# dkouzoup/ms-eetc

Hardware: NVIDIA B200
Metric: OCP solves/sec (batched, 1/2/4/8 B200) vs CasADi+IPOPT on host cores (higher is better)
Workload: dtype f64

## Files before the change

ms-eetc_b200/csrc/mseetc_b200.cu:

```cuda
#include <cuda_runtime.h>
#include <cooperative_groups.h>

#include <algorithm>
#include <cstdio>
#include <limits>
#include <cstdlib>
#include <cstring>
#include <new>
#include <string>
#include <vector>

#include "../../include/mseetc_b200.h"
#include "variants.h"
#include "compact.cuh"
#include "table.cuh"

using namespace mseetc;

static_assert((int)MSEETC_PARAM_COUNT == (int)PAR_N, "parameter plane enum out of sync");
static_assert((int)MSEETC_P_MASS == (int)P_MASS, "parameter plane enum out of sync");

namespace {

thread_local std::string g_err;


#ifndef MS_MINB_TRIAL
#define MS_MINB_TRIAL 2
#endif
#ifndef MS_MINB_EVAL
#define MS_MINB_EVAL 2
#endif
#ifndef MS_MINB_STEP
#define MS_MINB_STEP 3
#endif
MS_CELL_KERNEL(k_cell_setup, 4, cell_setup(c, io, k, s))
MS_CELL_KERNEL(k_cell_init, 4, cell_init<false>(c, k, s))
MS_CELL_KERNEL(k_cell_trial_eval, MS_MINB_TRIAL, (cell_eval<false, true>(c, k, s)))
MS_CELL_KERNEL(k_cell_eval, MS_MINB_EVAL, (cell_eval<false, false>(c, k, s)))
MS_CELL_KERNEL(k_cell_step, MS_MINB_STEP, cell_step<false>(c, k, s))
MS_CELL_KERNEL(k_cell_extract, 4, cell_extract(c, io, k, s))

__global__ void __launch_bounds__(64) k_inst_setup(Ctx c, BatchIO io) {
    const int s = blockIdx.x * blockDim.x + threadIdx.x;
    if (s < c.cfg.S) inst_setup(c, io, s);
}
__global__ void __launch_bounds__(128) k_inst_profile(Ctx c, int useSmem) {
    extern __shared__ double prof_sm[];
    const int half = blockDim.x >> 1;
    const bool profileRole = (int)threadIdx.x >= half;
    const int col = profileRole ? (int)threadIdx.x - half : (int)threadIdx.x;
    const int s = blockIdx.x * half + col;
    if (s >= c.cfg.S) return;
    if (!profileRole) { inst_screen(c, s); return; }
    if (useSmem) inst_profile(c, s, prof_sm + col, prof_sm + (size_t)c.cfg.NK * half + col, half);
    else inst_profile(c, s);
}

#ifndef MS_RED_CL
#define MS_RED_CL 4
#endif
enum { RED_CL = MS_RED_CL, RED_WB = RED_W / RED_CL };
static_assert(RED_W % RED_CL == 0, "cluster size must divide the interleave factor");
__device__ __forceinline__ const double* cluster_peer(const double* p, unsigned rank) {
    return cooperative_groups::this_cluster().map_shared_rank(p, rank);
}
__device__ __forceinline__ void prefetch_instance_state(const Ctx& c, int s) {
    for (int f = 0; f < SD_N; ++f) asm volatile("prefetch.global.L1 [%0];" ::"l"(&c.D(f, s)));
    for (int f = 0; f < SI_N; ++f) asm volatile("prefetch.global.L1 [%0];" ::"l"(&c.I(f, s)));
}

__global__ void __cluster_dims__(RED_CL, 1, 1) __launch_bounds__(32 * RED_WB) k_inst_alpha(Ctx c, int* mirror) {
    namespace cg = cooperative_groups;
    cg::cluster_group cl = cg::this_cluster();
    if (mirror && blockIdx.x == 0 && threadIdx.x == 0) *mirror = *(volatile int*)c.done;
    __shared__ double sm[RED_WB][3][32];
    const unsigned rank = cl.block_rank();
    const int lane = threadIdx.x & 31, wl = threadIdx.x >> 5, w = (int)rank * RED_WB + wl;
    const int s = (blockIdx.x / RED_CL) * 32 + lane;
    const bool on = s < c.cfg.nInst && c.I(SI_PHASE, s) == PH_STEPPED;
    double acc[3] = {1.0, 1.0, 0.0};
    if (on) alpha_partials(c, s, c.I(SI_N_INT, s), w, RED_W, acc);
    if (on && rank == 0 && wl == 0) prefetch_instance_state(c, s);
    for (int f = 0; f < 3; ++f) sm[wl][f][lane] = acc[f];
    cl.sync();
    double tot[3] = {1.0, 1.0, 0.0};
    if (rank == 0 && wl == 0 && on) {
        for (int ww = 0; ww < RED_W; ++ww) {
            const double* q = cluster_peer(&sm[ww % RED_WB][0][lane], ww / RED_WB);
            tot[0] = fmin(tot[0], q[0]); tot[1] = fmin(tot[1], q[32]); tot[2] += q[64];
        }
    }
    cl.sync();
    if (rank == 0 && wl == 0 && on) inst_alpha(c, s, tot);
}

template <bool TRIAL>
__global__ void __cluster_dims__(RED_CL, 1, 1) __launch_bounds__(32 * RED_WB) k_inst_kkt(Ctx c) {
    namespace cg = cooperative_groups;
    cg::cluster_group cl = cg::this_cluster();
    __shared__ double sm[RED_WB][10][32];
    const unsigned rank = cl.block_rank();
    const int lane = threadIdx.x & 31, wl = threadIdx.x >> 5, w = (int)rank * RED_WB + wl;
    const int s = (blockIdx.x / RED_CL) * 32 + lane;
    const bool on = s < c.cfg.nInst && c.I(SI_PHASE, s) == (TRIAL ? PH_TRIAL : PH_EVAL);
    KktAcc acc;
    kkt_init(acc);
    if (on) kkt_partials(c, s, c.I(SI_N_INT, s), ((c.I(SI_PARITY, s) != 0) != TRIAL) ? WS_IT1 : WS_IT0, w, RED_W, acc);
    if (on && rank == 0 && wl == 0) prefetch_instance_state(c, s);
    sm[wl][0][lane] = acc.th; sm[wl][1][lane] = acc.fo; sm[wl][2][lane] = acc.slog; sm[wl][3][lane] = acc.sdamp;
    sm[wl][4][lane] = acc.zsum; sm[wl][5][lane] = acc.ysum; sm[wl][6][lane] = acc.dinf; sm[wl][7][lane] = acc.pinf;
    sm[wl][8][lane] = acc.cmin; sm[wl][9][lane] = acc.cmax;
    cl.sync();
    KktAcc tot;
    kkt_init(tot);
    const bool lead = rank == 0 && wl == 0 && on;
    if (lead) {
        for (int ww = 0; ww < RED_W; ++ww) {
            const double* q = cluster_peer(&sm[ww % RED_WB][0][lane], ww / RED_WB);
            KktAcc o;
            o.th = q[0]; o.fo = q[32]; o.slog = q[64]; o.sdamp = q[96];
            o.zsum = q[128]; o.ysum = q[160]; o.dinf = q[192]; o.pinf = q[224];
            o.cmin = q[256]; o.cmax = q[288];
            kkt_combine(tot, o);
        }
    }
    cl.sync();
    if (lead) {
        if (TRIAL) {
            const double sums[4] = {tot.th, tot.fo, tot.slog, tot.sdamp};
            inst_decide(c, s, sums);
        } else count_cells(c, 4, c.I(SI_N_INT, s) + 1);
        inst_kkt(c, s, tot);
    }
}

template <int BS, int DEPTH, bool BULK>
__global__ void __launch_bounds__(BS) k_step(Ctx c) {
    extern __shared__ __align__(128) double ring[];
    const int s = blockIdx.x * BS + threadIdx.x;
    if (s >= c.cfg.S) return;
    const int lane = threadIdx.x & 31, warp = threadIdx.x >> 5;
    const bool active = s < c.cfg.nInst && c.I(SI_PHASE, s) == PH_FACTOR;
    double* wring = ring + (size_t)warp * ((DEPTH + 1) * RING_NF_MAX * 32);
    if (BULK) {
        const unsigned mask = __ballot_sync(0xffffffffu, active);
        if (!active) return;
        const int N = c.I(SI_N_INT, s);
        if (__all_sync(mask, N == __shfl_sync(mask, N, __ffs((int)mask) - 1))) {
            unsigned long long* bars = reinterpret_cast<unsigned long long*>(ring + (size_t)(BS / 32) * ((DEPTH + 1) * RING_NF_MAX * 32))
                                       + (size_t)warp * 2 * (DEPTH + 1);
            BulkRing<BwdFields, DEPTH> fb;
            BulkRing<FwdFields, DEPTH> ff;
            fb.setup(wring, bars, mask, lane);
            ff.setup(wring, bars + (DEPTH + 1), mask, lane);
            inst_step_warp(c, s, mask, fb, ff);
            return;
        }
    }
    if (!active) return;
    RingFetch<BwdFields, 32, DEPTH> fb;
    fb.sm = wring + lane;
    RingFetch<FwdFields, 32, DEPTH> ff;
    ff.sm = wring + lane;
    inst_step(c, s, fb, ff);
}

#ifndef MS_PIT_PF
#define MS_PIT_PF 3
#endif
template <int SL, int G, int DEPTH>
__global__ void __launch_bounds__(SL * G) k_step_pit(Ctx c, int* fallbackCount) {
    extern __shared__ __align__(128) double pit_sm[];
    constexpr int BS = SL * G;
    double* ring = pit_sm;
    double* shbase = pit_sm + (size_t)(DEPTH + 1) * RING_NF_MAX * BS;
    int* flags = reinterpret_cast<int*>(shbase + (size_t)G * SH_N * SL);
    const int col = threadIdx.x % SL, l = threadIdx.x / SL;
    const int s = blockIdx.x * SL + col;
    const bool active = s < c.cfg.nInst && c.I(SI_PHASE, s) == PH_FACTOR;
    if (!__syncthreads_or(active)) return;
    PitShare sh{shbase, flags, SL};
    PitLane t;
    t.s = s; t.col = col; t.l = l; t.G = G;
    t.N = active ? c.I(SI_N_INT, s) : 2;
    t.mu = active ? c.D(SD_MU, s) : 0.1;
    t.delta = 0.0;
    const double dlast = active ? c.D(SD_DELTA_LAST, s) : 0.0;
    pit_chunk(t.N, G, l, t.kLo, t.kHi);
    if (active) pit_read_reference(c, t);
    if (l == 0) flags[col] = 0;
    RingFetch<BwdFields, BS, DEPTH, MS_PIT_PF> fb;
    fb.sm = ring + threadIdx.x;
    constexpr int FDEPTH = ((DEPTH + 1) * BwdFields::NF) / FwdFields::NF - 1;
    RingFetch<FwdFields, BS, FDEPTH, 2 * MS_PIT_PF> ff;
    ff.sm = ring + threadIdx.x;
    double delta = 0.0;
    bool pending = active, failed = false, fallback = false;
    int why = 0;
    for (int tries = 0; tries < 40; ++tries) {
        if (!__syncthreads_or(pending)) break;
        t.delta = delta;
        if (pending) {
            if (l == 0) count_cells(c, 2, t.N);
            pit_phase_a(c, t, sh, fb);
        }
        __syncthreads();
        if (pending && l == 0) pit_value_chain(sh, col, G);
        __syncthreads();
        if (pending) pit_phase_c(c, t, sh, fb);
        __syncthreads();
        const int f = flags[col];
        __syncthreads();
        if (l == 0) flags[col] = 0;
        if (pending) {
            if (f & PIT_SCAN_FAILED) { fallback = true; pending = false; why = f; }
            else if (f & PIT_BAD_INERTIA) {
                if (l == 0) c.I(SI_NREG, s) += 1;
                delta = pit_next_delta(delta, dlast);
                if (delta > 1e40) { failed = true; pending = false; }
            } else pending = false;
        }
    }
    if (pending) failed = true;
    if (__syncthreads_or(fallback)) {
        if (fallback && l == 0) {
            atomicAdd(fallbackCount, 1);
            if (why & PIT_ELEM_FAILED) atomicAdd(fallbackCount + 1, 1);
            if (why & PIT_APPLY_FAILED) atomicAdd(fallbackCount + 2, 1);
            if (why & PIT_INCONSISTENT) atomicAdd(fallbackCount + 3, 1);
            inst_step(c, s, fb, ff);
        }
        __syncthreads();
    }
    const bool go = active && !fallback && !failed;
    if (failed && l == 0) finish(c, s, ST_STEP_FAILED);
    if (go && l == 0) {
        pit_state_chain(sh, col, G);
        count_cells(c, 3, t.N);
        if (delta > 0.0) c.D(SD_DELTA_LAST, s) = delta;
        c.D(SD_DELTA, s) = delta;
    }
    __syncthreads();
    if (go) pit_phase_f(c, t, sh, ff);
    if (go && l == 0) { c.I(SI_FACT, s) = 1; c.I(SI_PHASE, s) = PH_STEPPED; }
}

__global__ void k_loop_cond(cudaGraphConditionalHandle handle, int* counters, int n, int maxTicks) {
    const int tick = ++counters[53];
    cudaGraphSetConditional(handle, (*(volatile int*)counters < n && tick <= maxTicks) ? 1u : 0u);
}

__global__ void __launch_bounds__(128) k_cell_table(TableIO io, LossMapDev lm) {
    const size_t total = (size_t)(io.Nmax + 1) * io.n;
    for (size_t idx = (size_t)blockIdx.x * 128 + threadIdx.x; idx < total; idx += (size_t)gridDim.x * 128)
        cell_table(io, lm, (int)(idx % (io.Nmax + 1)), (int)(idx / (io.Nmax + 1)));
// ... 315 lines not shown
        static const int stepDepth = []() { const char* e = getenv("MSEETC_STEP_DEPTH"); return e ? atoi(e) : 16; }();
        if (depth >= 16 && stepDepth >= 16 && !stepBulk) { depth = 16; stepKernel = k_step<32, 16, false>; }
        else if (depth >= 8) { depth = 8; stepKernel = stepBulk ? k_step<32, 8, true> : k_step<32, 8, false>; }
        else { depth = 4; stepKernel = k_step<32, 4, false>; }
    } else {
        if (depth >= 4) { depth = 4; stepKernel = k_step<64, 4, false>; }
        else if (depth >= 2) { depth = 2; stepKernel = k_step<64, 2, false>; }
        else { depth = 1; stepKernel = k_step<64, 1, false>; }
    }
    size_t ringBytes = (size_t)(depth + 1) * slotBytes + (size_t)(ib / 32) * 2 * (depth + 1) * sizeof(unsigned long long);
    static const int stepSmemKb = []() { const char* e = getenv("MSEETC_STEP_SMEM_KB"); return e ? atoi(e) : -1; }();
    {
        const int bps = blocksPerSm < 1 ? 1 : blocksPerSm;
        const size_t pad = stepSmemKb >= 0 ? (size_t)stepSmemKb * 1024 : (size_t)228 * 1024 / (bps + 1) + 1024;
        if (pad > ringBytes && pad <= (size_t)227 * 1024) ringBytes = pad;
    }
    cudaFuncSetAttribute(stepKernel, cudaFuncAttributeMaxDynamicSharedMemorySize, 227 * 1024);
    void (*pitKernel)(Ctx, int*) = nullptr;
    int pitThreads = 0, pitSL = 8;
    size_t pitBytes = 0;
    int lanesNow = h->sweep_lanes;
    if (lanesNow == 0) {
        const int Nmax = p.n_intervals_max;
        lanesNow = Nmax >= 1024 ? 32 : Nmax >= 96 ? 16 : Nmax >= 48 ? 8 : 1;
        if (lanesNow > 1 && lanesNow < 32 && g.S > 4096) lanesNow = 1;
    }
    h->last_lanes = lanesNow;
    if (lanesNow > 1) {
        const int G = lanesNow;
        pitSL = (G == 32) ? 8 : 16;
        if (G == 8) pitKernel = k_step_pit<16, 8, 1>;
        else if (G == 16) pitKernel = k_step_pit<16, 16, 1>;
        else pitKernel = k_step_pit<8, 32, 1>;
        pitThreads = pitSL * G;
        pitBytes = sizeof(double) * ((size_t)2 * RING_NF_MAX * pitThreads + (size_t)G * SH_N * pitSL) + sizeof(int) * pitSL;
        cudaFuncSetAttribute(pitKernel, cudaFuncAttributeMaxDynamicSharedMemorySize, 227 * 1024);
    }
    int launches = 0;
    cudaError_t e;
    for (int i = 0; i < NCLS; ++i) { h->ms[i] = 0.0; h->launches[i] = 0; h->cells[i] = 0; }
    std::vector<int> evClass;
    auto begin = [&](int cls) {
        h->launches[cls] += 1;
        ++launches;
        if (!h->profiling) return;
        const size_t need = 2 * (evClass.size() + 1);
        while (h->ev.size() < need) { cudaEvent_t x; cudaEventCreate(&x); h->ev.push_back(x); }
        cudaEventRecord(h->ev[2 * evClass.size()], st);
    };
    auto end = [&](int cls) {
        if (!h->profiling) return;
        cudaEventRecord(h->ev[2 * evClass.size() + 1], st);
        evClass.push_back(cls);
    };
    e = cudaMemsetAsync(c.done, 0, 256, st);
    if (e != cudaSuccess) return cuda_fail(e, "cudaMemsetAsync");
    e = cudaMemsetAsync(c.si, 0, sizeof(int) * (size_t)SI_N * g.S, st);
    if (e != cudaSuccess) return cuda_fail(e, "cudaMemsetAsync");
    const unsigned rgrid = (unsigned)(g.S / 32);
    begin(CLS_MISC); k_inst_setup<<<igrid, ib, 0, st>>>(c, io); end(CLS_MISC);
    begin(CLS_MISC); k_cell_setup<<<cgrid, 128, 0, st>>>(c, io); end(CLS_MISC);
    if (g.initMode || (tmin && g.energy)) {
        size_t profBytes = (size_t)2 * g.NK * ib * sizeof(double);
        if (profBytes > (size_t)200 * 1024 / (blocksPerSm < 1 ? 1 : blocksPerSm)) profBytes = 0;
        if (profBytes) cudaFuncSetAttribute(k_inst_profile, cudaFuncAttributeMaxDynamicSharedMemorySize, 227 * 1024);
        begin(CLS_MISC); k_inst_profile<<<igrid, 2 * ib, profBytes, st>>>(c, profBytes ? 1 : 0); end(CLS_MISC);
    }
    begin(CLS_MISC);
    if (intl) launch_variant(c.irk ? VK_INIT_INTL_IRK : VK_INIT_INTL, cgrid, st, c, io);
    else if (dyn) launch_variant(VK_INIT_DYN, cgrid, st, c, io); else k_cell_init<<<cgrid, 128, 0, st>>>(c, io);
    end(CLS_MISC);
    const int maxTicks = 3 * p.max_iterations + 100;
    int tick = 0;
    begin(CLS_EVAL);
    if (intl) launch_variant(c.irk ? VK_EVAL_INTL_IRK : VK_EVAL_INTL, gridIrk, st, c, io);
    else if (c.irk) launch_variant(dyn ? VK_EVAL_DYN_IRK : VK_EVAL_IRK, gridIrk, st, c, io);
    else if (dyn) launch_variant(VK_EVAL_DYN, gridEval, st, c, io); else k_cell_eval<<<gridEval, 128, 0, st>>>(c, io);
    end(CLS_EVAL);
    begin(CLS_KKT); k_inst_kkt<false><<<rgrid * RED_CL, 32 * RED_WB, 0, st>>>(c); end(CLS_KKT);
    static const bool compactOn = []() { const char* e = getenv("MSEETC_COMPACT"); return !e || atoi(e) != 0; }();
    h->last_compactions = 0;
    static const int graphEnv = []() { const char* e = getenv("MSEETC_GRAPH"); return e ? atoi(e) : -1; }();
    const bool useGraph = !h->profiling && (graphEnv == 1 || (graphEnv != 0 && g.S <= 256 && !tmin));
    auto tick_kernels = [&](cudaStream_t s0, int* mirror, bool prof) {
        if (prof) begin(CLS_STEP);
        if (pitKernel) pitKernel<<<(unsigned)(g.S / pitSL), pitThreads, pitBytes, s0>>>(c, c.done + 48);
        else stepKernel<<<igrid, ib, ringBytes, s0>>>(c);
        if (prof) end(CLS_STEP);
        if (prof) begin(CLS_CSTEP);
        if (intl) launch_variant(VK_STEP_INTL, pgrid(2), s0, c, io);
        else if (dyn) launch_variant(VK_STEP_DYN, gridStep, s0, c, io); else k_cell_step<<<gridStep, 128, 0, s0>>>(c, io);
        if (prof) end(CLS_CSTEP);
        if (prof) begin(CLS_ALPHA);
        k_inst_alpha<<<rgrid * RED_CL, 32 * RED_WB, 0, s0>>>(c, mirror);
        if (prof) end(CLS_ALPHA);
        if (prof) begin(CLS_TRIAL);
        if (intl) launch_variant(c.irk ? VK_TRIAL_INTL_IRK : VK_TRIAL_INTL, gridIrk, s0, c, io);
        else if (c.irk) launch_variant(dyn ? VK_TRIAL_DYN_IRK : VK_TRIAL_IRK, gridIrk, s0, c, io);
        else if (dyn) launch_variant(VK_TRIAL_DYN, gridTrial, s0, c, io); else k_cell_trial_eval<<<gridTrial, 128, 0, s0>>>(c, io);
        if (prof) end(CLS_TRIAL);
        if (prof) begin(CLS_DECIDE);
        k_inst_kkt<true><<<rgrid * RED_CL, 32 * RED_WB, 0, s0>>>(c);
        if (prof) end(CLS_DECIDE);
    };
    if (useGraph) {
        unsigned char key[sizeof h->loop_key];
        memset(key, 0, sizeof key);
        memcpy(key, &c, sizeof(Ctx));
        memcpy(key + sizeof(Ctx), &io, sizeof(BatchIO));
        int stPrio = 0;
        cudaStreamGetPriority(st, &stPrio);
        const int extra[4] = {lanesNow * 4 + (dyn ? 1 : 0), stPrio, maxTicks, n};
        memcpy(key + sizeof(Ctx) + sizeof(BatchIO), extra, sizeof extra);
        if (!h->loop_exec || memcmp(key, h->loop_key, sizeof key) != 0) {
            if (h->loop_exec) { cudaGraphExecDestroy(h->loop_exec); h->loop_exec = nullptr; }
            if (h->loop_graph) { cudaGraphDestroy(h->loop_graph); h->loop_graph = nullptr; }
            if (h->cap_stream && stPrio != h->cap_prio) { cudaStreamDestroy(h->cap_stream); h->cap_stream = nullptr; }
            if (!h->cap_stream) {
                if ((e = cudaStreamCreateWithPriority(&h->cap_stream, cudaStreamNonBlocking, stPrio)) != cudaSuccess) return cuda_fail(e, "cudaStreamCreateWithPriority");
                h->cap_prio = stPrio;
            }
            if ((e = cudaGraphCreate(&h->loop_graph, 0)) != cudaSuccess) return cuda_fail(e, "cudaGraphCreate");
            cudaGraphConditionalHandle cond;
            if ((e = cudaGraphConditionalHandleCreate(&cond, h->loop_graph, 1, cudaGraphCondAssignDefault)) != cudaSuccess) return cuda_fail(e, "cudaGraphConditionalHandleCreate");
            cudaGraphNodeParams np = {cudaGraphNodeTypeConditional};
            np.conditional.handle = cond;
            np.conditional.type = cudaGraphCondTypeWhile;
            np.conditional.size = 1;
            cudaGraphNode_t node;
            if ((e = cudaGraphAddNode(&node, h->loop_graph, nullptr, 0, &np)) != cudaSuccess) return cuda_fail(e, "cudaGraphAddNode(conditional)");
            cudaGraph_t bodyGraph = np.conditional.phGraph_out[0];
            cudaStream_t cs = h->cap_stream;
            if ((e = cudaStreamBeginCaptureToGraph(cs, bodyGraph, nullptr, nullptr, 0, cudaStreamCaptureModeRelaxed)) != cudaSuccess) return cuda_fail(e, "cudaStreamBeginCaptureToGraph");
            tick_kernels(cs, nullptr, false);
            k_loop_cond<<<1, 1, 0, cs>>>(cond, c.done, n, maxTicks);
            cudaError_t le = cudaGetLastError();
            e = cudaStreamEndCapture(cs, nullptr);
            if (le != cudaSuccess) return cuda_fail(le, "tick capture");
            if (e != cudaSuccess) return cuda_fail(e, "cudaStreamEndCapture");
            if ((e = cudaGraphInstantiate(&h->loop_exec, h->loop_graph, 0)) != cudaSuccess) return cuda_fail(e, "cudaGraphInstantiate");
            memcpy(h->loop_key, key, sizeof key);
        }
        if ((e = cudaGraphLaunch(h->loop_exec, st)) != cudaSuccess) return cuda_fail(e, "cudaGraphLaunch");
    } else {
        for (;;) {
            tick_kernels(st, h->done_host_dev + 32 + tick % 4, true);
            ++tick;
            if (tick >= maxTicks) break;
            const int slot = (tick - 1) % 4;
            cudaEventRecord(h->poll_ev[slot], st);
            if (tick >= 3) {
                const int old = (tick - 3) % 4;
                e = cudaEventSynchronize(h->poll_ev[old]);
                if (e != cudaSuccess) return cuda_fail(e, "solver kernels");
                const int doneLag = h->done_host[32 + old];
                if (doneLag >= n) break;
                if (compactOn && h->compaction && !intl && g.S >= 256 && doneLag > 0 && tick % 4 == 0) {
                    const int activeUb = n - doneLag;
                    k_compact_plan<<<1, 1024, 0, st>>>(c);
                    k_compact_extract<<<cgrid, 128, 0, st>>>(c, io);
                    k_compact_move<<<(unsigned)(((size_t)activeUb * g.NK + 127) / 128), 128, 0, st>>>(c);
                    k_compact_finish<<<(unsigned)((n + 127) / 128), 128, 0, st>>>(c);
                    k_compact_state<<<(unsigned)((activeUb + 127) / 128), 128, 0, st>>>(c);
                    launches += 5;
                    ++h->last_compactions;
                }
            }
        }
    }
    begin(CLS_MISC); k_cell_extract<<<cgrid, 128, 0, st>>>(c, io); end(CLS_MISC);
    if (intl && lam_out) launch_variant(c.irk ? VK_LAM_INTL_IRK : VK_LAM_INTL, cgrid, st, c, io);
    e = cudaGetLastError();
    if (e != cudaSuccess) return cuda_fail(e, "kernel launch");
    e = cudaMemcpyAsync(h->done_host, c.done, 256, cudaMemcpyDeviceToHost, st);
    if (e != cudaSuccess) return cuda_fail(e, "cudaMemcpyAsync(counters)");
    e = cudaStreamSynchronize(st);
    if (e != cudaSuccess) return cuda_fail(e, "solver kernels");
    {
        const unsigned long long* cnt = (const unsigned long long*)((const char*)h->done_host + 64);
        h->cells[CLS_TRIAL] = (long long)cnt[0];
        h->cells[CLS_DECIDE] = (long long)cnt[0];
        h->cells[CLS_EVAL] = (long long)cnt[4];
        h->cells[CLS_STEP] = (long long)cnt[1];
        h->cells[CLS_CSTEP] = (long long)cnt[3] + (long long)(cnt[3] / (unsigned long long)(p.n_intervals_max));
        h->cells[CLS_ALPHA] = h->cells[CLS_CSTEP];
        h->cells[CLS_KKT] = (long long)cnt[4];
        h->cells[CLS_MISC] = 0;
        h->last_fallbacks = (long long)h->done_host[48];
        for (int i = 0; i < 3; ++i) h->fallback_why[i] = h->done_host[49 + i];
    }
    for (size_t i = 0; i < evClass.size(); ++i) {
        float ms = 0.f;
        cudaEventElapsedTime(&ms, h->ev[2 * i], h->ev[2 * i + 1]);
        h->ms[evClass[i]] += ms;
    }
    h->ev_class = evClass;
    if (useGraph) {
        tick = h->done_host[53];
        for (int cls : {CLS_STEP, CLS_CSTEP, CLS_ALPHA, CLS_TRIAL, CLS_DECIDE}) h->launches[cls] = tick;
        launches += 6 * tick;
    }
    h->last_ticks = tick;
    h->last_launches = launches;
    h->last_moves = h->done_host[54];
    return 0;
}

int mseetc_discretize_tracks(int32_t n_tracks, const double* length, const int32_t* n_int, const int32_t* lim_off, const double* lim_pos,
                             const double* lim_val, const int32_t* grd_off, const double* grd_pos, const double* grd_val, const int32_t* crv_off,
                             const double* crv_pos, const double* crv_val, const int32_t* out_off, double* pos_nodes, double* limit_nodes,
                             double* grad_nodes, double* curv_nodes, int32_t* error) {
    if (n_tracks < 1 || !length || !n_int || !lim_off || !lim_pos || !lim_val || !grd_off || !grd_pos || !grd_val || !crv_off || !crv_pos ||
        !crv_val || !out_off || !pos_nodes || !limit_nodes || !grad_nodes || !curv_nodes || !error)
        return fail(-1, "mseetc_discretize_tracks: bad argument");
    std::vector<double> brk, grid;
    for (int t = 0; t < n_tracks; ++t) {
        const int N = n_int[t];
        const double L = length[t];
        error[t] = 0;
        brk.clear();
        brk.insert(brk.end(), lim_pos + lim_off[t], lim_pos + lim_off[t + 1]);
        brk.insert(brk.end(), grd_pos + grd_off[t], grd_pos + grd_off[t + 1]);
        brk.insert(brk.end(), crv_pos + crv_off[t], crv_pos + crv_off[t + 1]);
        std::sort(brk.begin(), brk.end());
        brk.erase(std::unique(brk.begin(), brk.end()), brk.end());
        const int M = (int)brk.size();
        const int nuni = N + 1 - (M - 1);
        if (N < 1 || nuni < 2) { error[t] = 1; continue; }
        grid.assign(brk.begin(), brk.end());
        const double step = L / (nuni - 1);
        for (int j = 0; j < nuni; ++j) grid.push_back(j == nuni - 1 ? L : j * step);
        std::sort(grid.begin(), grid.end());
        grid.erase(std::unique(grid.begin(), grid.end()), grid.end());
        if ((int)grid.size() != N + 1) { error[t] = 1; continue; }
        double* po = pos_nodes + out_off[t] + t;
        double* lo = limit_nodes + out_off[t] + t;
        double* go = grad_nodes + out_off[t] + t;
        double* co = curv_nodes + out_off[t] + t;
        int il = lim_off[t], ig = grd_off[t], ic = crv_off[t];
        const double nan = std::numeric_limits<double>::quiet_NaN();
        for (int k = 0; k <= N; ++k) {
            const double x = grid[k];
            while (il + 1 < lim_off[t + 1] && lim_pos[il + 1] <= x) ++il;
            while (ig + 1 < grd_off[t + 1] && grd_pos[ig + 1] <= x) ++ig;
            while (ic + 1 < crv_off[t + 1] && crv_pos[ic + 1] <= x) ++ic;
            po[k] = x;
            lo[k] = (lim_off[t + 1] > lim_off[t] && lim_pos[il] <= x) ? lim_val[il] : nan;
            go[k] = (grd_off[t + 1] > grd_off[t] && grd_pos[ig] <= x) ? grd_val[ig] : nan;
// ... 113 lines not shown
```

ms-eetc_b200/csrc/variants.h:

```cpp
#pragma once
#include <cuda_runtime.h>
#include "io.cuh"

namespace mseetc {

enum VariantKernel {
    VK_INIT_DYN, VK_EVAL_DYN, VK_TRIAL_DYN, VK_STEP_DYN,
    VK_EVAL_IRK, VK_EVAL_DYN_IRK, VK_TRIAL_IRK, VK_TRIAL_DYN_IRK,
    VK_INIT_INTL, VK_EVAL_INTL, VK_TRIAL_INTL, VK_STEP_INTL, VK_LAM_INTL,
    VK_INIT_INTL_IRK, VK_EVAL_INTL_IRK, VK_TRIAL_INTL_IRK, VK_LAM_INTL_IRK
};
void launch_variant_dyn(int which, unsigned grid, cudaStream_t st, const Ctx& c, const BatchIO& io);
void launch_variant_irk(int which, unsigned grid, cudaStream_t st, const Ctx& c, const BatchIO& io);
void launch_variant_intl(int which, unsigned grid, cudaStream_t st, const Ctx& c, const BatchIO& io);
void launch_variant_intl_irk(int which, unsigned grid, cudaStream_t st, const Ctx& c, const BatchIO& io);
inline void launch_variant(int which, unsigned grid, cudaStream_t st, const Ctx& c, const BatchIO& io) {
    if (which <= VK_STEP_DYN) launch_variant_dyn(which, grid, st, c, io);
    else if (which <= VK_TRIAL_DYN_IRK) launch_variant_irk(which, grid, st, c, io);
    else if (which <= VK_LAM_INTL) launch_variant_intl(which, grid, st, c, io);
    else launch_variant_intl_irk(which, grid, st, c, io);
}
void launch_eval_interval_irk(int n, int numSteps, int numApprox, const double* in, double* out, const IrkTab* irk, cudaStream_t st);

#define MS_CELL_KERNEL(NAME, MINB, CALL)                                        \
    __global__ void __launch_bounds__(128, MINB) NAME(Ctx c, BatchIO io) {      \
        const size_t total = (size_t)c.cfg.NK * c.cfg.S;                        \
        const size_t stride = (size_t)gridDim.x * 128;                          \
        for (size_t idx = (size_t)blockIdx.x * 128 + threadIdx.x; idx < total; idx += stride) { \
            const int s = (int)(idx % c.cfg.S);                                 \
            const int k = (int)(idx / c.cfg.S);                                 \
            CALL;                                                               \
        }                                                                       \
    }

}
```

ms-eetc_b200/csrc/variants_dyn.cu:

```cuda
#include "variants.h"

namespace mseetc {
namespace {
#ifndef MS_MINB_STEP
#define MS_MINB_STEP 3
#endif
MS_CELL_KERNEL(k_cell_init_dyn, 2, cell_init<true>(c, k, s))
MS_CELL_KERNEL(k_cell_trial_eval_dyn, 2, (cell_eval<true, true>(c, k, s)))
MS_CELL_KERNEL(k_cell_eval_dyn, 2, (cell_eval<true, false>(c, k, s)))
MS_CELL_KERNEL(k_cell_step_dyn, MS_MINB_STEP, cell_step<true>(c, k, s))
}

void launch_variant_dyn(int which, unsigned grid, cudaStream_t st, const Ctx& c, const BatchIO& io) {
    switch (which) {
        case VK_INIT_DYN: k_cell_init_dyn<<<grid, 128, 0, st>>>(c, io); break;
        case VK_EVAL_DYN: k_cell_eval_dyn<<<grid, 128, 0, st>>>(c, io); break;
        case VK_TRIAL_DYN: k_cell_trial_eval_dyn<<<grid, 128, 0, st>>>(c, io); break;
        case VK_STEP_DYN: k_cell_step_dyn<<<grid, 128, 0, st>>>(c, io); break;
        default: break;
    }
}

}
```

ms-eetc_b200/csrc/variants_intl.cu:

```cuda
#include "variants.h"

#ifndef MS_PART
#define MS_PART 0
#endif

namespace mseetc {
void launch_variant_intl_eval(int which, unsigned grid, cudaStream_t st, const Ctx& c, const BatchIO& io);

#if MS_PART == 0
namespace {
MS_CELL_KERNEL(k_cell_init_intl, 1, (cell_init<true, true>(c, k, s)))
MS_CELL_KERNEL(k_cell_step_intl, 2, (cell_step<true, true>(c, k, s)))
MS_CELL_KERNEL(k_cell_lam_intl, 1, cell_fix_time_multiplier_intl<false>(c, io, k, s))
}

void launch_variant_intl(int which, unsigned grid, cudaStream_t st, const Ctx& c, const BatchIO& io) {
    switch (which) {
        case VK_INIT_INTL: k_cell_init_intl<<<grid, 128, 0, st>>>(c, io); break;
        case VK_STEP_INTL: k_cell_step_intl<<<grid, 128, 0, st>>>(c, io); break;
        case VK_LAM_INTL: k_cell_lam_intl<<<grid, 128, 0, st>>>(c, io); break;
        default: launch_variant_intl_eval(which, grid, st, c, io); break;
    }
}
#else
namespace {
MS_CELL_KERNEL(k_cell_trial_eval_intl, 1, (cell_eval<true, true, false, true>(c, k, s)))
MS_CELL_KERNEL(k_cell_eval_intl, 1, (cell_eval<true, false, false, true>(c, k, s)))
}

void launch_variant_intl_eval(int which, unsigned grid, cudaStream_t st, const Ctx& c, const BatchIO& io) {
    switch (which) {
        case VK_EVAL_INTL: k_cell_eval_intl<<<grid, 128, 0, st>>>(c, io); break;
        case VK_TRIAL_INTL: k_cell_trial_eval_intl<<<grid, 128, 0, st>>>(c, io); break;
        default: break;
    }
}
#endif

}
```

ms-eetc_b200/csrc/variants_intl_irk.cu:

```cuda
#include "variants.h"

#ifndef MS_PART
#define MS_PART 0
#endif

namespace mseetc {
void launch_variant_intl_irk_eval(int which, unsigned grid, cudaStream_t st, const Ctx& c, const BatchIO& io);
void launch_variant_intl_irk_trial(int which, unsigned grid, cudaStream_t st, const Ctx& c, const BatchIO& io);

#if MS_PART == 0
namespace {
MS_CELL_KERNEL(k_cell_init_intl_irk, 1, (cell_init<true, true, true>(c, k, s)))
MS_CELL_KERNEL(k_cell_lam_intl_irk, 1, cell_fix_time_multiplier_intl<true>(c, io, k, s))
}

void launch_variant_intl_irk(int which, unsigned grid, cudaStream_t st, const Ctx& c, const BatchIO& io) {
    switch (which) {
        case VK_INIT_INTL_IRK: k_cell_init_intl_irk<<<grid, 128, 0, st>>>(c, io); break;
        case VK_LAM_INTL_IRK: k_cell_lam_intl_irk<<<grid, 128, 0, st>>>(c, io); break;
        case VK_EVAL_INTL_IRK: launch_variant_intl_irk_eval(which, grid, st, c, io); break;
        default: launch_variant_intl_irk_trial(which, grid, st, c, io); break;
    }
}
#elif MS_PART == 1
namespace {
MS_CELL_KERNEL(k_cell_eval_intl_irk, 1, (cell_eval<true, false, true, true>(c, k, s)))
}
void launch_variant_intl_irk_eval(int, unsigned grid, cudaStream_t st, const Ctx& c, const BatchIO& io) {
    k_cell_eval_intl_irk<<<grid, 128, 0, st>>>(c, io);
}
#else
namespace {
MS_CELL_KERNEL(k_cell_trial_eval_intl_irk, 1, (cell_eval<true, true, true, true>(c, k, s)))
}
void launch_variant_intl_irk_trial(int, unsigned grid, cudaStream_t st, const Ctx& c, const BatchIO& io) {
    k_cell_trial_eval_intl_irk<<<grid, 128, 0, st>>>(c, io);
}
#endif

}
```

ms-eetc_b200/csrc/variants_irk.cu:

```cuda
#include "variants.h"

namespace mseetc {
namespace {
MS_CELL_KERNEL(k_cell_trial_eval_irk, 1, (cell_eval<false, true, true>(c, k, s)))
MS_CELL_KERNEL(k_cell_trial_eval_dyn_irk, 1, (cell_eval<true, true, true>(c, k, s)))
MS_CELL_KERNEL(k_cell_eval_irk, 1, (cell_eval<false, false, true>(c, k, s)))
MS_CELL_KERNEL(k_cell_eval_dyn_irk, 1, (cell_eval<true, false, true>(c, k, s)))

__global__ void k_eval_interval_irk(int n, int numSteps, int numApprox, const double* in, double* out, const IrkTab* irk) {
    const int i = blockIdx.x * blockDim.x + threadIdx.x;
    eval_interval_point<true>(i, n, numSteps, numApprox, in, out, irk);
}
}

void launch_variant_irk(int which, unsigned grid, cudaStream_t st, const Ctx& c, const BatchIO& io) {
    switch (which) {
        case VK_EVAL_IRK: k_cell_eval_irk<<<grid, 128, 0, st>>>(c, io); break;
        case VK_EVAL_DYN_IRK: k_cell_eval_dyn_irk<<<grid, 128, 0, st>>>(c, io); break;
        case VK_TRIAL_IRK: k_cell_trial_eval_irk<<<grid, 128, 0, st>>>(c, io); break;
        case VK_TRIAL_DYN_IRK: k_cell_trial_eval_dyn_irk<<<grid, 128, 0, st>>>(c, io); break;
        default: break;
    }
}

void launch_eval_interval_irk(int n, int numSteps, int numApprox, const double* in, double* out, const IrkTab* irk, cudaStream_t st) {
    k_eval_interval_irk<<<(n + 127) / 128, 128, 0, st>>>(n, numSteps, numApprox, in, out, irk);
}

}
```

Baseline: 114,900.

## Enable programmatic dependent launch and poll host-mapped completion mirror

Launches the per-tick solver kernels through cudaLaunchKernelEx with programmatic stream serialization, and has every kernel call griddepcontrol.wait then launch_dependents at entry. The next kernel's launch can then overlap the tail of the previous one while data dependencies still hold. The host loop stops recording and synchronizing on events (unless an env var asks for it) and instead spins on a host-mapped mirror slot reset to -1, with cudaStreamQuery as a fallback. This trims per-tick host sync latency at the cost of busy polling and extra code paths; PDL is turned off for the step launch right after a compaction.

```diff
diff --git a/ms-eetc_b200/csrc/mseetc_b200.cu b/ms-eetc_b200/csrc/mseetc_b200.cu
--- a/ms-eetc_b200/csrc/mseetc_b200.cu
+++ b/ms-eetc_b200/csrc/mseetc_b200.cu
@@ -72,6 +72,8 @@
 
 __global__ void __cluster_dims__(RED_CL, 1, 1) __launch_bounds__(32 * RED_WB) k_inst_alpha(Ctx c, int* mirror) {
     namespace cg = cooperative_groups;
+    grid_dep_wait();
+    grid_dep_release();
     cg::cluster_group cl = cg::this_cluster();
     if (mirror && blockIdx.x == 0 && threadIdx.x == 0) *mirror = *(volatile int*)c.done;
     __shared__ double sm[RED_WB][3][32];
@@ -98,6 +100,8 @@
 template <bool TRIAL>
 __global__ void __cluster_dims__(RED_CL, 1, 1) __launch_bounds__(32 * RED_WB) k_inst_kkt(Ctx c) {
     namespace cg = cooperative_groups;
+    grid_dep_wait();
+    grid_dep_release();
     cg::cluster_group cl = cg::this_cluster();
     __shared__ double sm[RED_WB][10][32];
     const unsigned rank = cl.block_rank();
@@ -138,6 +142,8 @@
 template <int BS, int DEPTH, bool BULK>
 __global__ void __launch_bounds__(BS) k_step(Ctx c) {
     extern __shared__ __align__(128) double ring[];
+    grid_dep_wait();
+    grid_dep_release();
     const int s = blockIdx.x * BS + threadIdx.x;
     if (s >= c.cfg.S) return;
     const int lane = threadIdx.x & 31, warp = threadIdx.x >> 5;
@@ -172,6 +178,8 @@
 template <int SL, int G, int DEPTH>
 __global__ void __launch_bounds__(SL * G) k_step_pit(Ctx c, int* fallbackCount) {
     extern __shared__ __align__(128) double pit_sm[];
+    grid_dep_wait();
+    grid_dep_release();
     constexpr int BS = SL * G;
     double* ring = pit_sm;
     double* shbase = pit_sm + (size_t)(DEPTH + 1) * RING_NF_MAX * BS;
@@ -653,25 +661,30 @@
     h->last_compactions = 0;
     static const int graphEnv = []() { const char* e = getenv("MSEETC_GRAPH"); return e ? atoi(e) : -1; }();
     const bool useGraph = !h->profiling && (graphEnv == 1 || (graphEnv != 0 && g.S <= 256 && !tmin));
-    auto tick_kernels = [&](cudaStream_t s0, int* mirror, bool prof) {
+    static const bool pdlOn = []() { const char* e = getenv("MSEETC_PDL"); return !e || atoi(e) != 0; }();
+    auto tick_kernels = [&](cudaStream_t s0, int* mirror, bool prof, bool plainSweep) {
+        const bool pdl = pdlOn;
+        const dim3 rgridC(rgrid * RED_CL), rblock(32 * RED_WB);
         if (prof) begin(CLS_STEP);
-        if (pitKernel) pitKernel<<<(unsigned)(g.S / pitSL), pitThreads, pitBytes, s0>>>(c, c.done + 48);
-        else stepKernel<<<igrid, ib, ringBytes, s0>>>(c);
+        if (pitKernel) launch_k(pitKernel, dim3(g.S / pitSL), dim3(pitThreads), pitBytes, s0, pdl && !plainSweep, c, c.done + 48);
+        else launch_k(stepKernel, dim3(igrid), dim3(ib), ringBytes, s0, pdl && !plainSweep, c);
         if (prof) end(CLS_STEP);
         if (prof) begin(CLS_CSTEP);
-        if (intl) launch_variant(VK_STEP_INTL, pgrid(2), s0, c, io);
-        else if (dyn) launch_variant(VK_STEP_DYN, gridStep, s0, c, io); else k_cell_step<<<gridStep, 128, 0, s0>>>(c, io);
+        if (intl) launch_variant(VK_STEP_INTL, pgrid(2), s0, c, io, pdl);
+        else if (dyn) launch_variant(VK_STEP_DYN, gridStep, s0, c, io, pdl);
+        else launch_k(k_cell_step, dim3(gridStep), dim3(128), 0, s0, pdl, c, io);
         if (prof) end(CLS_CSTEP);
         if (prof) begin(CLS_ALPHA);
-        k_inst_alpha<<<rgrid * RED_CL, 32 * RED_WB, 0, s0>>>(c, mirror);
+        launch_k(k_inst_alpha, rgridC, rblock, 0, s0, pdl, c, mirror);
         if (prof) end(CLS_ALPHA);
         if (prof) begin(CLS_TRIAL);
-        if (intl) launch_variant(c.irk ? VK_TRIAL_INTL_IRK : VK_TRIAL_INTL, gridIrk, s0, c, io);
-        else if (c.irk) launch_variant(dyn ? VK_TRIAL_DYN_IRK : VK_TRIAL_IRK, gridIrk, s0, c, io);
-        else if (dyn) launch_variant(VK_TRIAL_DYN, gridTrial, s0, c, io); else k_cell_trial_eval<<<gridTrial, 128, 0, s0>>>(c, io);
+        if (intl) launch_variant(c.irk ? VK_TRIAL_INTL_IRK : VK_TRIAL_INTL, gridIrk, s0, c, io, pdl);
+        else if (c.irk) launch_variant(dyn ? VK_TRIAL_DYN_IRK : VK_TRIAL_IRK, gridIrk, s0, c, io, pdl);
+        else if (dyn) launch_variant(VK_TRIAL_DYN, gridTrial, s0, c, io, pdl);
+        else launch_k(k_cell_trial_eval, dim3(gridTrial), dim3(128), 0, s0, pdl, c, io);
         if (prof) end(CLS_TRIAL);
         if (prof) begin(CLS_DECIDE);
-        k_inst_kkt<true><<<rgrid * RED_CL, 32 * RED_WB, 0, s0>>>(c);
+        launch_k(k_inst_kkt<true>, rgridC, rblock, 0, s0, pdl, c);
         if (prof) end(CLS_DECIDE);
     };
     if (useGraph) {
@@ -703,7 +716,7 @@
             cudaGraph_t bodyGraph = np.conditional.phGraph_out[0];
             cudaStream_t cs = h->cap_stream;
             if ((e = cudaStreamBeginCaptureToGraph(cs, bodyGraph, nullptr, nullptr, 0, cudaStreamCaptureModeRelaxed)) != cudaSuccess) return cuda_fail(e, "cudaStreamBeginCaptureToGraph");
-            tick_kernels(cs, nullptr, false);
+            tick_kernels(cs, nullptr, false, false);
             k_loop_cond<<<1, 1, 0, cs>>>(cond, c.done, n, maxTicks);
             cudaError_t le = cudaGetLastError();
             e = cudaStreamEndCapture(cs, nullptr);
@@ -714,17 +727,29 @@
         }
         if ((e = cudaGraphLaunch(h->loop_exec, st)) != cudaSuccess) return cuda_fail(e, "cudaGraphLaunch");
     } else {
+        static const bool pollEvent = []() { const char* e = getenv("MSEETC_POLL_EVENT"); return e && atoi(e) != 0; }();
+        volatile int* ring = h->done_host + 32;
+        bool compacted = false;
         for (;;) {
-            tick_kernels(st, h->done_host_dev + 32 + tick % 4, true);
+            ring[tick % 4] = -1;
+            tick_kernels(st, h->done_host_dev + 32 + tick % 4, true, compacted);
+            compacted = false;
             ++tick;
             if (tick >= maxTicks) break;
             const int slot = (tick - 1) % 4;
-            cudaEventRecord(h->poll_ev[slot], st);
+            if (pollEvent) cudaEventRecord(h->poll_ev[slot], st);
             if (tick >= 3) {
                 const int old = (tick - 3) % 4;
-                e = cudaEventSynchronize(h->poll_ev[old]);
-                if (e != cudaSuccess) return cuda_fail(e, "solver kernels");
-                const int doneLag = h->done_host[32 + old];
+                if (pollEvent) {
+                    e = cudaEventSynchronize(h->poll_ev[old]);
+                    if (e != cudaSuccess) return cuda_fail(e, "solver kernels");
+                }
+                while (ring[old] < 0) {
+                    e = cudaStreamQuery(st);
+                    if (e == cudaSuccess && ring[old] < 0) return fail(-7, "mseetc_solve_batch: completion mirror not written");
+                    if (e != cudaSuccess && e != cudaErrorNotReady) return cuda_fail(e, "solver kernels");
+                }
+                const int doneLag = ring[old];
                 if (doneLag >= n) break;
                 if (compactOn && h->compaction && !intl && g.S >= 256 && doneLag > 0 && tick % 4 == 0) {
                     const int activeUb = n - doneLag;
@@ -735,6 +760,7 @@
                     k_compact_state<<<(unsigned)((activeUb + 127) / 128), 128, 0, st>>>(c);
                     launches += 5;
                     ++h->last_compactions;
+                    compacted = true;
                 }
             }
         }
diff --git a/ms-eetc_b200/csrc/variants.h b/ms-eetc_b200/csrc/variants.h
--- a/ms-eetc_b200/csrc/variants.h
+++ b/ms-eetc_b200/csrc/variants.h
@@ -10,20 +10,43 @@
     VK_INIT_INTL, VK_EVAL_INTL, VK_TRIAL_INTL, VK_STEP_INTL, VK_LAM_INTL,
     VK_INIT_INTL_IRK, VK_EVAL_INTL_IRK, VK_TRIAL_INTL_IRK, VK_LAM_INTL_IRK
 };
-void launch_variant_dyn(int which, unsigned grid, cudaStream_t st, const Ctx& c, const BatchIO& io);
-void launch_variant_irk(int which, unsigned grid, cudaStream_t st, const Ctx& c, const BatchIO& io);
-void launch_variant_intl(int which, unsigned grid, cudaStream_t st, const Ctx& c, const BatchIO& io);
-void launch_variant_intl_irk(int which, unsigned grid, cudaStream_t st, const Ctx& c, const BatchIO& io);
-inline void launch_variant(int which, unsigned grid, cudaStream_t st, const Ctx& c, const BatchIO& io) {
-    if (which <= VK_STEP_DYN) launch_variant_dyn(which, grid, st, c, io);
-    else if (which <= VK_TRIAL_DYN_IRK) launch_variant_irk(which, grid, st, c, io);
-    else if (which <= VK_LAM_INTL) launch_variant_intl(which, grid, st, c, io);
-    else launch_variant_intl_irk(which, grid, st, c, io);
+__device__ __forceinline__ void grid_dep_wait() {
+#if defined(__CUDA_ARCH__)
+    asm volatile("griddepcontrol.wait;" ::: "memory");
+#endif
+}
+__device__ __forceinline__ void grid_dep_release() {
+#if defined(__CUDA_ARCH__)
+    asm volatile("griddepcontrol.launch_dependents;" ::: "memory");
+#endif
+}
+template <typename... KArgs, typename... Args>
+inline cudaError_t launch_k(void (*kern)(KArgs...), dim3 grid, dim3 block, size_t smem, cudaStream_t st, bool pdl, Args... args) {
+    cudaLaunchAttribute at[1];
+    at[0].id = cudaLaunchAttributeProgrammaticStreamSerialization;
+    at[0].val.programmaticStreamSerializationAllowed = 1;
+    cudaLaunchConfig_t cfg = {};
+    cfg.gridDim = grid; cfg.blockDim = block; cfg.dynamicSmemBytes = smem; cfg.stream = st;
+    cfg.attrs = at; cfg.numAttrs = pdl ? 1 : 0;
+    return cudaLaunchKernelEx(&cfg, kern, args...);
+}
+
+void launch_variant_dyn(int which, unsigned grid, cudaStream_t st, const Ctx& c, const BatchIO& io, bool pdl);
+void launch_variant_irk(int which, unsigned grid, cudaStream_t st, const Ctx& c, const BatchIO& io, bool pdl);
+void launch_variant_intl(int which, unsigned grid, cudaStream_t st, const Ctx& c, const BatchIO& io, bool pdl);
+void launch_variant_intl_irk(int which, unsigned grid, cudaStream_t st, const Ctx& c, const BatchIO& io, bool pdl);
+inline void launch_variant(int which, unsigned grid, cudaStream_t st, const Ctx& c, const BatchIO& io, bool pdl = false) {
+    if (which <= VK_STEP_DYN) launch_variant_dyn(which, grid, st, c, io, pdl);
+    else if (which <= VK_TRIAL_DYN_IRK) launch_variant_irk(which, grid, st, c, io, pdl);
+    else if (which <= VK_LAM_INTL) launch_variant_intl(which, grid, st, c, io, pdl);
+    else launch_variant_intl_irk(which, grid, st, c, io, pdl);
 }
 void launch_eval_interval_irk(int n, int numSteps, int numApprox, const double* in, double* out, const IrkTab* irk, cudaStream_t st);
 
 #define MS_CELL_KERNEL(NAME, MINB, CALL)                                        \
     __global__ void __launch_bounds__(128, MINB) NAME(Ctx c, BatchIO io) {      \
+        grid_dep_wait();                                                        \
+        grid_dep_release();                                                     \
         const size_t total = (size_t)c.cfg.NK * c.cfg.S;                        \
         const size_t stride = (size_t)gridDim.x * 128;                          \
         for (size_t idx = (size_t)blockIdx.x * 128 + threadIdx.x; idx < total; idx += stride) { \
diff --git a/ms-eetc_b200/csrc/variants_dyn.cu b/ms-eetc_b200/csrc/variants_dyn.cu
--- a/ms-eetc_b200/csrc/variants_dyn.cu
+++ b/ms-eetc_b200/csrc/variants_dyn.cu
@@ -11,12 +11,12 @@
 MS_CELL_KERNEL(k_cell_step_dyn, MS_MINB_STEP, cell_step<true>(c, k, s))
 }
 
-void launch_variant_dyn(int which, unsigned grid, cudaStream_t st, const Ctx& c, const BatchIO& io) {
+void launch_variant_dyn(int which, unsigned grid, cudaStream_t st, const Ctx& c, const BatchIO& io, bool pdl) {
     switch (which) {
-        case VK_INIT_DYN: k_cell_init_dyn<<<grid, 128, 0, st>>>(c, io); break;
-        case VK_EVAL_DYN: k_cell_eval_dyn<<<grid, 128, 0, st>>>(c, io); break;
-        case VK_TRIAL_DYN: k_cell_trial_eval_dyn<<<grid, 128, 0, st>>>(c, io); break;
-        case VK_STEP_DYN: k_cell_step_dyn<<<grid, 128, 0, st>>>(c, io); break;
+        case VK_INIT_DYN: launch_k(k_cell_init_dyn, grid, 128, 0, st, pdl, c, io); break;
+        case VK_EVAL_DYN: launch_k(k_cell_eval_dyn, grid, 128, 0, st, pdl, c, io); break;
+        case VK_TRIAL_DYN: launch_k(k_cell_trial_eval_dyn, grid, 128, 0, st, pdl, c, io); break;
+        case VK_STEP_DYN: launch_k(k_cell_step_dyn, grid, 128, 0, st, pdl, c, io); break;
         default: break;
     }
 }
diff --git a/ms-eetc_b200/csrc/variants_intl.cu b/ms-eetc_b200/csrc/variants_intl.cu
--- a/ms-eetc_b200/csrc/variants_intl.cu
+++ b/ms-eetc_b200/csrc/variants_intl.cu
@@ -5,7 +5,7 @@
 #endif
 
 namespace mseetc {
-void launch_variant_intl_eval(int which, unsigned grid, cudaStream_t st, const Ctx& c, const BatchIO& io);
+void launch_variant_intl_eval(int which, unsigned grid, cudaStream_t st, const Ctx& c, const BatchIO& io, bool pdl);
 
 #if MS_PART == 0
 namespace {
@@ -14,12 +14,12 @@
 MS_CELL_KERNEL(k_cell_lam_intl, 1, cell_fix_time_multiplier_intl<false>(c, io, k, s))
 }
 
-void launch_variant_intl(int which, unsigned grid, cudaStream_t st, const Ctx& c, const BatchIO& io) {
+void launch_variant_intl(int which, unsigned grid, cudaStream_t st, const Ctx& c, const BatchIO& io, bool pdl) {
     switch (which) {
-        case VK_INIT_INTL: k_cell_init_intl<<<grid, 128, 0, st>>>(c, io); break;
-        case VK_STEP_INTL: k_cell_step_intl<<<grid, 128, 0, st>>>(c, io); break;
-        case VK_LAM_INTL: k_cell_lam_intl<<<grid, 128, 0, st>>>(c, io); break;
-        default: launch_variant_intl_eval(which, grid, st, c, io); break;
+        case VK_INIT_INTL: launch_k(k_cell_init_intl, grid, 128, 0, st, pdl, c, io); break;
+        case VK_STEP_INTL: launch_k(k_cell_step_intl, grid, 128, 0, st, pdl, c, io); break;
+        case VK_LAM_INTL: launch_k(k_cell_lam_intl, grid, 128, 0, st, pdl, c, io); break;
+        default: launch_variant_intl_eval(which, grid, st, c, io, pdl); break;
     }
 }
 #else
@@ -28,10 +28,10 @@
 MS_CELL_KERNEL(k_cell_eval_intl, 1, (cell_eval<true, false, false, true>(c, k, s)))
 }
 
-void launch_variant_intl_eval(int which, unsigned grid, cudaStream_t st, const Ctx& c, const BatchIO& io) {
+void launch_variant_intl_eval(int which, unsigned grid, cudaStream_t st, const Ctx& c, const BatchIO& io, bool pdl) {
     switch (which) {
-        case VK_EVAL_INTL: k_cell_eval_intl<<<grid, 128, 0, st>>>(c, io); break;
-        case VK_TRIAL_INTL: k_cell_trial_eval_intl<<<grid, 128, 0, st>>>(c, io); break;
+        case VK_EVAL_INTL: launch_k(k_cell_eval_intl, grid, 128, 0, st, pdl, c, io); break;
+        case VK_TRIAL_INTL: launch_k(k_cell_trial_eval_intl, grid, 128, 0, st, pdl, c, io); break;
         default: break;
     }
 }
diff --git a/ms-eetc_b200/csrc/variants_intl_irk.cu b/ms-eetc_b200/csrc/variants_intl_irk.cu
--- a/ms-eetc_b200/csrc/variants_intl_irk.cu
+++ b/ms-eetc_b200/csrc/variants_intl_irk.cu
@@ -5,8 +5,8 @@
 #endif
 
 namespace mseetc {
-void launch_variant_intl_irk_eval(int which, unsigned grid, cudaStream_t st, const Ctx& c, const BatchIO& io);
-void launch_variant_intl_irk_trial(int which, unsigned grid, cudaStream_t st, const Ctx& c, const BatchIO& io);
+void launch_variant_intl_irk_eval(int which, unsigned grid, cudaStream_t st, const Ctx& c, const BatchIO& io, bool pdl);
+void launch_variant_intl_irk_trial(int which, unsigned grid, cudaStream_t st, const Ctx& c, const BatchIO& io, bool pdl);
 
 #if MS_PART == 0
 namespace {
@@ -14,27 +14,27 @@
 MS_CELL_KERNEL(k_cell_lam_intl_irk, 1, cell_fix_time_multiplier_intl<true>(c, io, k, s))
 }
 
-void launch_variant_intl_irk(int which, unsigned grid, cudaStream_t st, const Ctx& c, const BatchIO& io) {
+void launch_variant_intl_irk(int which, unsigned grid, cudaStream_t st, const Ctx& c, const BatchIO& io, bool pdl) {
     switch (which) {
-        case VK_INIT_INTL_IRK: k_cell_init_intl_irk<<<grid, 128, 0, st>>>(c, io); break;
-        case VK_LAM_INTL_IRK: k_cell_lam_intl_irk<<<grid, 128, 0, st>>>(c, io); break;
-        case VK_EVAL_INTL_IRK: launch_variant_intl_irk_eval(which, grid, st, c, io); break;
-        default: launch_variant_intl_irk_trial(which, grid, st, c, io); break;
+        case VK_INIT_INTL_IRK: launch_k(k_cell_init_intl_irk, grid, 128, 0, st, pdl, c, io); break;
+        case VK_LAM_INTL_IRK: launch_k(k_cell_lam_intl_irk, grid, 128, 0, st, pdl, c, io); break;
+        case VK_EVAL_INTL_IRK: launch_variant_intl_irk_eval(which, grid, st, c, io, pdl); break;
+        default: launch_variant_intl_irk_trial(which, grid, st, c, io, pdl); break;
     }
 }
 #elif MS_PART == 1
 namespace {
 MS_CELL_KERNEL(k_cell_eval_intl_irk, 1, (cell_eval<true, false, true, true>(c, k, s)))
 }
-void launch_variant_intl_irk_eval(int, unsigned grid, cudaStream_t st, const Ctx& c, const BatchIO& io) {
-    k_cell_eval_intl_irk<<<grid, 128, 0, st>>>(c, io);
+void launch_variant_intl_irk_eval(int, unsigned grid, cudaStream_t st, const Ctx& c, const BatchIO& io, bool pdl) {
+    launch_k(k_cell_eval_intl_irk, grid, 128, 0, st, pdl, c, io);
 }
 #else
 namespace {
 MS_CELL_KERNEL(k_cell_trial_eval_intl_irk, 1, (cell_eval<true, true, true, true>(c, k, s)))
 }
-void launch_variant_intl_irk_trial(int, unsigned grid, cudaStream_t st, const Ctx& c, const BatchIO& io) {
-    k_cell_trial_eval_intl_irk<<<grid, 128, 0, st>>>(c, io);
+void launch_variant_intl_irk_trial(int, unsigned grid, cudaStream_t st, const Ctx& c, const BatchIO& io, bool pdl) {
+    launch_k(k_cell_trial_eval_intl_irk, grid, 128, 0, st, pdl, c, io);
 }
 #endif
 
diff --git a/ms-eetc_b200/csrc/variants_irk.cu b/ms-eetc_b200/csrc/variants_irk.cu
--- a/ms-eetc_b200/csrc/variants_irk.cu
+++ b/ms-eetc_b200/csrc/variants_irk.cu
@@ -13,12 +13,12 @@
 }
 }
 
-void launch_variant_irk(int which, unsigned grid, cudaStream_t st, const Ctx& c, const BatchIO& io) {
+void launch_variant_irk(int which, unsigned grid, cudaStream_t st, const Ctx& c, const BatchIO& io, bool pdl) {
     switch (which) {
-        case VK_EVAL_IRK: k_cell_eval_irk<<<grid, 128, 0, st>>>(c, io); break;
-        case VK_EVAL_DYN_IRK: k_cell_eval_dyn_irk<<<grid, 128, 0, st>>>(c, io); break;
-        case VK_TRIAL_IRK: k_cell_trial_eval_irk<<<grid, 128, 0, st>>>(c, io); break;
-        case VK_TRIAL_DYN_IRK: k_cell_trial_eval_dyn_irk<<<grid, 128, 0, st>>>(c, io); break;
+        case VK_EVAL_IRK: launch_k(k_cell_eval_irk, grid, 128, 0, st, pdl, c, io); break;
+        case VK_EVAL_DYN_IRK: launch_k(k_cell_eval_dyn_irk, grid, 128, 0, st, pdl, c, io); break;
+        case VK_TRIAL_IRK: launch_k(k_cell_trial_eval_irk, grid, 128, 0, st, pdl, c, io); break;
+        case VK_TRIAL_DYN_IRK: launch_k(k_cell_trial_eval_dyn_irk, grid, 128, 0, st, pdl, c, io); break;
         default: break;
     }
 }
```

New measurement: 112,700, median of 6. -1.9%, worse.
